# davidesantangelo/krep

Hardware: AMD Instinct MI355X
Metric: GB/s scanned (literal scan, match offsets produced), haystack resident in HBM (higher is better)
Workload: dtype u8; 1 GPU; literal8: 8-byte case-sensitive literal 'Sherlock', ~1e-4 matches/byte, offsets tracked; 32 GiB per GPU (BASELINE.json configs[1]); pattern=Sherlock, bytes_per_gpu=34359738368, matches=3436005, parallelism=contiguous shards x1, start-offset ownership, 1 RCCL all-reduce of counts

## Files before the change

### krep_amd/csrc/kg_literal_dma.hip

```cpp
#include <hip/hip_runtime.h>
#include <algorithm>
#include <atomic>
#include <cstdlib>
#include "kg_common.h"
#include "kg_device.h"
#include "kg_internal.h"
#include "kg_tickets.h"

namespace kg {

namespace {

constexpr u32 kDmaPark = 80;
constexpr u32 kDmaRing = 2u * kSegBytes;
constexpr u32 kDmaTail = 256u;
constexpr u32 kDmaWaveLds = kDmaRing + kDmaTail;
constexpr u32 kOpHits = 768;
constexpr u32 kOpTk = 32;
static_assert(kOpHits * 4u + kOpTk * 12u <= kDmaPark * 44u, "the one-pass mode's static LDS stays within the staging mode's (two workgroups per CU)");
static_assert(kOpTk <= 64u, "one lane per parked ticket picks its prefix up");
}
uint32_t lit_dma_one_pass_list() { return kOpHits; }

template <int KIND, bool MASKED, bool CI, bool ONEP>
__global__ __launch_bounds__(kBlock, 2) void lit_scan_dma(const LitArgs a, u64 *__restrict__ agg, const u64 *__restrict__ pref, const u64 n_tickets)
{
    extern __shared__ __attribute__((aligned(16))) uint8_t d_smem[];
    __shared__ u64 s_info_all[kWavesPerBlk][ONEP ? 1u : kDmaPark];
    __shared__ __attribute__((aligned(16))) unsigned short s_slots_all[kWavesPerBlk][ONEP ? 8u : kDmaPark * 16u];
    __shared__ u32 s_unit_all[kWavesPerBlk][ONEP ? 1u : kDmaPark];
    __shared__ u32 s_hits_all[kWavesPerBlk][ONEP ? kOpHits : 1u];
    __shared__ u32 s_tk_all[kWavesPerBlk][ONEP ? 3u * kOpTk : 1u];
    const u32 lane = lane_id();
    const u32 wave = __builtin_amdgcn_readfirstlane(threadIdx.x >> 6);
    if (ONEP && wave == 0)
    {
        u64 r = 1;
        if (lane == 0)
            r = __hip_atomic_fetch_add(&a.ctr->pad[0], 1ull, __ATOMIC_RELAXED, __HIP_MEMORY_SCOPE_AGENT);
        if (rfl64(r) == 0ull)
        {
            tk_resolve(agg, const_cast<u64 *>(pref), n_tickets, a.ctr, lane);
            return;
        }
    }
    u32 *s_hits = s_hits_all[wave];
    u32 *s_tk = s_tk_all[wave];
    uint8_t *ring = d_smem + wave * kDmaWaveLds;
    uint8_t *tailb = ring + kDmaRing;
    u64 *s_info = s_info_all[wave];
    unsigned short *s_slots = s_slots_all[wave];
    u32 *s_unit = s_unit_all[wave];
    const u32 ring_lds = (u32)(size_t)(__attribute__((address_space(3))) uint8_t *)ring;

    const bool want_pos = (a.flags & F_POS) != 0;
    const bool ww = (a.flags & F_WW) != 0;
    const u64 hi_match = (a.own_hi < a.text_len - a.m + 1) ? a.own_hi : (a.text_len - a.m + 1);
    constexpr u64 kUnitBytes = (u64)kRoundsBig * kSegBytes;
    const u64 n_units = a.num_tiles * kWavesPerBlk;

    const bool park = want_pos && a.stage_cap >= 16u && a.stage_cap <= 128u && (a.stage_cap & 7u) == 0u && n_units < (1ull << 32);
    const u32 park_max = park ? kDmaPark * 16u / a.stage_cap : 0u;
    u32 n_park = 0;
    auto flush_parked = [&]() __attribute__((always_inline)) {
        for (u32 i = lane; i < n_park; i += 64u)
        {
            const u64 u = s_unit[i];
            a.unitinfo[u] = s_info[i];
            if (s_info[i] & kUiCountMask)
            {
                uint4 *dst = reinterpret_cast<uint4 *>(reinterpret_cast<unsigned short *>(a.stage) + u * (u64)a.stage_cap);
                const uint4 *src = reinterpret_cast<const uint4 *>(&s_slots[i * a.stage_cap]);
                const u32 c = (u32)(s_info[i] & kUiCountMask), nv = ((c < a.stage_cap ? c : a.stage_cap) + 7u) >> 3;
                for (u32 q = 0; q < nv; ++q)
                    dst[q] = src[q];
            }
        }
        n_park = 0;
    };

    const u32 tk_units = a.upt ? a.upt : 1u;
    u64 static_next = (u64)blockIdx.x * kWavesPerBlk + wave;
    auto next_ticket = [&]() -> u64 {
        if (a.upt)
        {
            return wave_fetch_add(&a.ctr->ticket, 1ull, lane) * (u64)a.upt;
        }
        const u64 u = static_next;
        static_next += (u64)gridDim.x * kWavesPerBlk;
        return u;
    };
    auto issue_round = [&](u64 seg, u32 buf) -> bool {
        if (seg + kSegBytes > a.text_len)
            return false;
        const uint8_t *src = a.text + seg + lane * 16u;
        uint8_t *dst = ring + buf * kSegBytes;
#pragma unroll
        for (int j = 0; j < kCells; ++j)
            __builtin_amdgcn_global_load_lds((const __attribute__((address_space(1))) void *)(src + j * kCellBytes),
                                             (__attribute__((address_space(3))) void *)(dst + j * kCellBytes), 16, 0, 2 );
        return true;
    };
    auto issue_tail = [&](u64 at) -> bool {
        if (at + kDmaTail > a.text_len)
            return false;
        __builtin_amdgcn_global_load_lds((const __attribute__((address_space(1))) void *)(a.text + at + lane * 4u),
                                         (__attribute__((address_space(3))) void *)tailb, 4, 0, 0);
        return true;
    };

    u32 hp = 0;
    u32 used = 0;
    u32 n_tkp = 0;
    bool overflowed = false;
    auto hwrap = [](const u32 x) -> u32 { return x >= kOpHits ? x - kOpHits : x; };
    auto flush_records = [&](const u32 n_out) __attribute__((always_inline)) {
        u64 pfx = 0;
        if (lane < n_out)
            pfx = tk_wait_prefix_lane(pref, (u64)s_tk[3u * lane], a.ctr);
        for (u32 i = 0; i < n_out; ++i)
        {
            const u32 t = __builtin_amdgcn_readfirstlane(s_tk[3u * i]), cnt = __builtin_amdgcn_readfirstlane(s_tk[3u * i + 1u]),
                      at = __builtin_amdgcn_readfirstlane(s_tk[3u * i + 2u]);
            const u64 first = ((u64)(u32)__builtin_amdgcn_readlane((u32)(pfx >> 32), i) << 32) | (u32)__builtin_amdgcn_readlane((u32)pfx, i);
            const u64 tbase = a.global_base + a.anchor + (u64)t * ((u64)tk_units * kUnitBytes);
            const u32 pad = (u32)(first & 7ull);
            for (u32 q = lane; q < cnt + pad; q += 64u)
            {
                if (q < pad)
                    continue;
                const u32 e = q - pad;
                const u64 idx = first + e;
                if (idx < a.pos_cap)
                {
                    const u64 st = tbase + s_hits[hwrap(at + e)], en = st + a.m;
                    typedef u32 u32x4 __attribute__((ext_vector_type(4)));
                    const u32x4 rec = {(u32)st, (u32)(st >> 32), (u32)en, (u32)(en >> 32)};
                    __builtin_nontemporal_store(rec, reinterpret_cast<u32x4 *>(a.positions + 2 * idx));
                }
            }
            used -= cnt;
        }
        if (n_out < n_tkp)
        {
            const u32 t = s_tk[3u * n_out], cnt = s_tk[3u * n_out + 1u], at = s_tk[3u * n_out + 2u];
            if (lane == 0)
            {
                s_tk[0] = t;
                s_tk[1] = cnt;
                s_tk[2] = at;
            }
        }
        n_tkp -= n_out;
    };

    u64 acc_total = 0;
    u32 pf_cells = 0;
    u32 wcnt = 0;
    auto stage_hit = [&](u64 unit, u32 idx, u32 rel) __attribute__((always_inline)) {
        if (ONEP)
        {
            if (idx < kOpHits - used)
                s_hits[hwrap(hp + idx)] = rel;
        }
        else if (idx < a.stage_cap)
        {
            unsigned short *slot = park ? &s_slots[n_park * a.stage_cap] : reinterpret_cast<unsigned short *>(a.stage) + unit * (u64)a.stage_cap;
            slot[idx] = (unsigned short)rel;
        }
    };
    auto publish = [&](u64 unit) __attribute__((always_inline)) {
        if (ONEP)
            return;
        acc_total += wcnt;
        if (want_pos)
        {
            if (lane == 0)
            {
                const u64 info = (u64)wcnt | (wcnt ? (kLnHead | kLnTail) : 0ull);
                if (park)
                {
                    s_info[n_park] = info;
                    s_unit[n_park] = (u32)unit;
                }
                else
                    a.unitinfo[unit] = info;
                if (wcnt > a.stage_cap)
                {
                    atomicAdd(&a.ctr->overflow_units, 1ull);
                    atomicMax(&a.ctr->max_unit_count, (u64)wcnt);
                }
            }
            if (park && ++n_park == park_max)
                flush_parked();
        }
        wcnt = 0;
    };
    auto end_ticket = [&](u32 t) __attribute__((always_inline)) {
        if (lane == 0)
            __hip_atomic_store(&agg[t], (u64)wcnt | kTkReady, __ATOMIC_RELAXED, __HIP_MEMORY_SCOPE_AGENT);
        u32 fresh = 0;
        if (wcnt > kOpHits - used)
            overflowed = true;
        else if (wcnt)
        {
            if (lane == 0)
            {
                s_tk[3u * n_tkp] = t;
                s_tk[3u * n_tkp + 1u] = wcnt;
                s_tk[3u * n_tkp + 2u] = hp;
            }
            ++n_tkp;
            hp = hwrap(hp + wcnt);
            used += wcnt;
            fresh = 1;
        }
        wcnt = 0;
        if ((n_tkp == kOpTk || used > kOpHits / 2u) && n_tkp > fresh)
            flush_records(n_tkp - fresh);
    };
    auto exact = [&](u32 A0, u32 A4) -> bool {
        const u32 e0 = CI ? (A0 | a.l0) : A0;
        bool h = (KIND == 4 && MASKED) ? (((e0 ^ a.p0) & a.k0) == 0u) : (e0 == a.p0);
        if (KIND >= 8)
        {
            const u32 e4 = CI ? (A4 | a.l1) : A4;
            h = h && ((KIND == 8 && MASKED) ? (((e4 ^ a.p1) & a.k1) == 0u) : (e4 == a.p1));
        }
        return h;
    };
    auto owned = [&](u64 p) -> bool { return p >= a.own_lo && p < hi_match && !(p >= a.excl_lo && p < a.excl_hi); };
    auto word_ok = [&](u64 p) -> bool {
        if (p > 0 && p != a.ww_exempt_left && is_wordc(a.text[p - 1]))
            return false;
        if (p + a.m < a.text_len && is_wordc(a.text[p + a.m]))
            return false;
        return true;
    };
    auto boundary = [&](u64 seg_prev, u64 unit, u32 r_prev, u32 c0, u32 c1, u32 n0, u32 n1) __attribute__((always_inline)) {
        {
            const u32 f = 0x01010101u * ((CI ? (a.p0 | 0x20u) : a.p0) & 0xffu);
            const u32 y0 = (CI ? (c0 | 0x20202020u) : c0) ^ f, y1 = (CI ? (c1 | 0x20202020u) : c1) ^ f;
            if (((((y0 - 0x01010101u) & ~y0) | ((y1 - 0x01010101u) & ~y1)) & 0x80808080u) == 0u)
                return;
        }
        const u32 q = lane & 7u, sh = q & 3u;
        const bool up = (q >> 2) != 0u;
        const u32 lo = up ? c1 : c0, mid = up ? n0 : c1, hi = up ? n1 : n0;
        const u32 A0 = __builtin_amdgcn_alignbyte(mid, lo, sh), A4 = __builtin_amdgcn_alignbyte(hi, mid, sh);
        const u64 p = seg_prev + (kSegBytes - 8u) + q;
        bool h = lane < 8u && q + a.m > 8u && exact(A0, A4) && owned(p);
        if (ww && __ballot(h))
            h = h && word_ok(p);
        const u64 bm = __ballot(h);
        if (bm)
        {
            if (h && want_pos)
                stage_hit(unit, wcnt + mbcnt64(bm), r_prev * kSegBytes + (kSegBytes - 8u) + q);
            wcnt += (u32)__popcll(bm);
        }
    };

    u64 u0 = next_ticket();
    bool dma_cur = u0 < n_units && issue_round(a.anchor + u0 * kUnitBytes, 0u);
    while (u0 < n_units)
    {
        const u32 nun = (u32)((n_units - u0 < (u64)tk_units) ? (n_units - u0) : (u64)tk_units), nr = nun * (u32)kRoundsBig;
        const u64 tbase = a.anchor + u0 * kUnitBytes;
        u64 u_next = ~0ull;
        bool tail_ok = false;
        u32 c0 = 0, c1 = 0;
        bool deferred = false;
#pragma unroll 1
        for (u32 g = 0; g < nr; ++g)
        {
            const u64 seg = tbase + (u64)g * kSegBytes, unit = u0 + (g >> 2);
            const u32 r = g & 3u;
            bool dma_nx = false, tail_now = false;
            asm volatile("s_waitcnt lgkmcnt(0)" ::: "memory");
            if (g + 1u < nr)
                dma_nx = issue_round(seg + kSegBytes, (g + 1u) & 1u);
            else
            {
                u_next = next_ticket();
                if (u_next < n_units)
                    dma_nx = issue_round(a.anchor + u_next * kUnitBytes, (g + 1u) & 1u);
            }
            if (g + 2u == nr)
                tail_ok = tail_now = issue_tail(tbase + (u64)nr * kSegBytes);
            if (dma_cur)
            {
                if (dma_nx && tail_now)
                    asm volatile("s_waitcnt vmcnt(9)" ::: "memory");
                else if (dma_nx)
                    asm volatile("s_waitcnt vmcnt(8)" ::: "memory");
                else if (tail_now)
                    asm volatile("s_waitcnt vmcnt(1)" ::: "memory");
                else
                    asm volatile("s_waitcnt vmcnt(0)" ::: "memory");
            }
            const bool interior = seg >= a.own_lo && seg + kSegBytes <= hi_match && (seg + kSegBytes <= a.excl_lo || seg >= a.excl_hi);
            uint4 vv[kCells];
            uint2 nn[kCells];
            if (dma_cur)
            {
                typedef u32 v4 __attribute__((ext_vector_type(4)));
                typedef u32 v2 __attribute__((ext_vector_type(2)));
                const u32 addr = ring_lds + (g & 1u) * kSegBytes + lane * 16u;
                v4 x[kCells];
                v2 y[kCells];
#pragma unroll
                for (int j = 0; j < kCells; ++j)
                {
                    asm volatile("ds_read_b128 %0, %1 offset:%2" : "=v"(x[j]) : "v"(addr), "n"(j * (int)kCellBytes));
                    asm volatile("ds_read_b64 %0, %1 offset:%2" : "=v"(y[j]) : "v"(addr), "n"(j * (int)kCellBytes + 16));
                }
                asm volatile("s_waitcnt lgkmcnt(0)"
                             : "+v"(x[0]), "+v"(x[1]), "+v"(x[2]), "+v"(x[3]), "+v"(x[4]), "+v"(x[5]), "+v"(x[6]), "+v"(x[7]), "+v"(y[0]), "+v"(y[1]),
                               "+v"(y[2]), "+v"(y[3]), "+v"(y[4]), "+v"(y[5]), "+v"(y[6]), "+v"(y[7])
                             :
                             : "memory");
#pragma unroll
                for (int j = 0; j < kCells; ++j)
                {
                    vv[j] = make_uint4(x[j].x, x[j].y, x[j].z, x[j].w);
                    nn[j] = make_uint2(y[j].x, y[j].y);
                }
            }
            else
            {
#pragma unroll
                for (int j = 0; j < kCells; ++j)
                {
                    const W6 w = load_window_guarded(a.text, a.text_len, seg + (u64)j * kCellBytes + (u64)lane * 16u);
                    vv[j] = make_uint4(w.v[0], w.v[1], w.v[2], w.v[3]);
                    nn[j] = make_uint2(w.v[4], w.v[5]);
                }
            }
            if (deferred)
            {
                boundary(seg - kSegBytes, u0 + ((g - 1u) >> 2), ONEP ? g - 1u : (g - 1u) & 3u, c0, c1, __builtin_amdgcn_readfirstlane(vv[0].x),
                         __builtin_amdgcn_readfirstlane(vv[0].y));
                deferred = false;
                if (r == 0u)
                    publish(unit - 1u);
            }
            __builtin_amdgcn_sched_barrier(0);
#pragma unroll
            for (int j = 0; j < kCells; ++j)
            {
                const u64 lbase = seg + (u64)j * kCellBytes + (u64)lane * 16u;
                const u32 D[6] = {vv[j].x, vv[j].y, vv[j].z, vv[j].w, nn[j].x, nn[j].y};
                auto A = [&](int k) -> u32 {
                    return ((k & 3) == 0) ? D[k >> 2] : __builtin_amdgcn_alignbyte(D[(k >> 2) + 1], D[k >> 2], (u32)(k & 3));
                };
                u32 Dq[6];
#pragma unroll
                for (int w = 0; w < 6; ++w)
                    Dq[w] = CI ? (D[w] | 0x20202020u) : D[w];
                auto Aq = [&](int k) -> u32 {
                    return ((k & 3) == 0) ? Dq[k >> 2] : __builtin_amdgcn_alignbyte(Dq[(k >> 2) + 1], Dq[k >> 2], (u32)(k & 3));
                };
                const u32 p0q = CI ? (a.p0 | 0x20202020u) : a.p0;
                if (a.prefilter)
                {
                    u32 z = 0;
#pragma unroll
                    for (int w = 0; w < 4; ++w)
                    {
                        const u32 y = Dq[w] ^ a.prefilter;
                        z |= (y - 0x01010101u) & ~y;
                    }
                    if (!__ballot((z & 0x80808080u) != 0u))
                        continue;
                    ++pf_cells;
                }
                bool c[16];
                u64 any = 0;
#pragma unroll
                for (int k = 0; k < 16; ++k)
                {
                    const u32 x = Aq(k);
                    c[k] = (KIND == 4 && MASKED) ? (((x ^ p0q) & a.k0) == 0u) : (x == p0q);
                    any |= __ballot(c[k]);
                }
                if (!any)
                    continue;
                u32 m16 = 0;
#pragma unroll
                for (int k = 0; k < 16; ++k)
                    if (__ballot(c[k]))
                        m16 |= (c[k] && exact(A(k), A(k + 4))) ? (1u << k) : 0u;
                if (dma_cur && j == kCells - 1 && lane == 63u)
                    m16 &= (1u << (17u - a.m)) - 1u;
                if (!interior)
                {
                    auto clip = [&](u64 lo, u64 hi) -> u32 {
                        const u32 klo = lo > lbase ? (u32)((lo - lbase) < 16 ? (lo - lbase) : 16) : 0u;
                        const u32 khi = hi > lbase ? (u32)((hi - lbase) < 16 ? (hi - lbase) : 16) : 0u;
                        return khi > klo ? (((1u << khi) - 1u) & ~((1u << klo) - 1u)) : 0u;
                    };
                    m16 &= clip(a.own_lo, hi_match) & ~clip(a.excl_lo, a.excl_hi);
                }
                if (ww && __ballot(m16 != 0u))
                {
                    const u32 below = __shfl_up(D[3], 1);
                    auto pick = [&](u32 i) -> u32 {
                        const u32 q = i >> 2;
                        const u32 w = q == 0u ? below : q == 1u ? D[0] : q == 2u ? D[1] : q == 3u ? D[2] : q == 4u ? D[3] : q == 5u ? D[4] : D[5];
                        return (w >> (8u * (i & 3u))) & 0xffu;
                    };
                    const bool edge = dma_cur && j == kCells - 1 && lane == 63u;
                    u32 rest = m16;
                    while (rest)
                    {
                        const u32 k = __builtin_ctz(rest);
                        rest &= rest - 1u;
                        const u64 p = lbase + k;
                        bool bad;
                        if (edge || (lane == 0u && k == 0u))
                            bad = !word_ok(p);
                        else
                            bad = (p != a.ww_exempt_left && is_wordc(pick(k + 3u))) || is_wordc(pick(k + a.m + 4u));
                        if (bad)
                            m16 &= ~(1u << k);
                    }
                }
                if (!__ballot(m16 != 0u))
                    continue;
                const u32 cnt = __popc(m16);
                u32 idx = wcnt, tot = 0;
                auto plane = [&](int b) {
                    const u64 bm = __ballot((cnt >> b) & 1u);
                    idx += mbcnt64(bm) << b;
                    tot += (u32)__popcll(bm) << b;
                };
                plane(0);
                plane(1);
                if (__ballot(cnt > 3u))
                {
                    plane(2);
                    plane(3);
                    plane(4);
                }
                wcnt += tot;
                if (want_pos)
                {
                    const u32 rel0 = ((ONEP ? g : r) * (u32)kCells + (u32)j) * kCellBytes + lane * 16u;
                    u32 rest = m16;
                    while (rest)
                    {
                        const u32 k = __builtin_ctz(rest);
                        rest &= rest - 1u;
                        stage_hit(unit, idx++, rel0 + k);
                    }
                }
            }
            if (dma_cur)
            {
                c0 = __builtin_amdgcn_readlane(vv[kCells - 1].z, 63);
                c1 = __builtin_amdgcn_readlane(vv[kCells - 1].w, 63);
                deferred = true;
            }
            if (g + 1u == nr)
            {
                if (deferred)
                {
                    u32 n0 = 0, n1 = 0;
                    if (tail_ok)
                    {
                        typedef u32 v2 __attribute__((ext_vector_type(2)));
                        v2 t;
                        const u32 taddr = ring_lds + kDmaRing;
                        asm volatile("ds_read_b64 %0, %1\n\ts_waitcnt lgkmcnt(0)" : "=v"(t) : "v"(taddr) : "memory");
                        n0 = __builtin_amdgcn_readfirstlane(t.x);
                        n1 = __builtin_amdgcn_readfirstlane(t.y);
                    }
                    else
                    {
                        const W6 w = load_window_guarded(a.text, a.text_len, seg + kSegBytes);
                        n0 = __builtin_amdgcn_readfirstlane(w.v[0]);
                        n1 = __builtin_amdgcn_readfirstlane(w.v[1]);
                    }
                    boundary(seg, unit, ONEP ? g : r, c0, c1, n0, n1);
                    deferred = false;
                }
                if (ONEP)
                    end_ticket((u32)u0 / tk_units);
                else
                    publish(unit);
            }
            else if (!deferred && r == 3u)
                publish(unit);
            dma_cur = dma_nx;
        }
        u0 = u_next;
    }
    if (!ONEP && park && n_park)
        flush_parked();
    if (ONEP && n_tkp)
        flush_records(n_tkp);
    if (ONEP && overflowed && lane == 0)
        atomicAdd(&a.ctr->overflow_units, 1ull);
    if (lane == 0 && acc_total)
        atomicAdd(&a.ctr->total, acc_total);
    if (lane == 0 && pf_cells)
        atomicAdd(&a.ctr->candidates, (u64)pf_cells);
}

__global__ __launch_bounds__(256) void dma_byte_look(const uint8_t *text, u64 lo, u32 n_cells, u32 b4, u32 fold, unsigned long long *out)
{
    const u32 lane = lane_id();
    const u32 wave = blockIdx.x * 4u + (threadIdx.x >> 6), n_waves = gridDim.x * 4u;
    u32 cnt = 0;
    for (u32 c = wave; c < n_cells; c += n_waves)
    {
        const uint4 v = *reinterpret_cast<const uint4 *>(text + lo + (u64)c * kCellBytes + lane * 16u);
        const u32 d[4] = {v.x, v.y, v.z, v.w};
        u32 z = 0;
#pragma unroll
        for (int w = 0; w < 4; ++w)
        {
            const u32 y = (d[w] | fold) ^ b4;
            z |= (y - 0x01010101u) & ~y;
        }
        if (__ballot((z & 0x80808080u) != 0u))
            ++cnt;
    }
    if (lane == 0 && cnt)
        atomicAdd(out, (u64)cnt);
}
hipError_t launch_dma_byte_look(const uint8_t *text, uint64_t lo, uint32_t n_cells, uint32_t prefilter, bool ci, unsigned long long *out, hipStream_t st)
{
    hipLaunchKernelGGL(dma_byte_look, dim3(256), dim3(256), 0, st, text, (u64)lo, n_cells, prefilter, ci ? 0x20202020u : 0u, out);
    return hipGetLastError();
}

std::atomic<uint64_t> g_lit_dma_launches{0};
std::atomic<uint64_t> g_lit_dma1p_launches{0};
std::atomic<uint64_t> g_lit_dma1p_failovers{0};
int g_lit_dma1p_force_grid = 0;

template <int KIND, bool MASKED, bool CI, bool ONEP>
static hipError_t dma_launch4(const LitArgs &a, u64 *agg, const u64 *pref, u64 n_tickets, u32 num_cu, hipStream_t st)
{
    constexpr u32 lds = kWavesPerBlk * kDmaWaveLds;
    if (const hipError_t e = grant_dynamic_lds<&lit_scan_dma<KIND, MASKED, CI, ONEP>>((int)lds); e != hipSuccess)
        return e;
    static const u32 bpc = [] { const char *e = getenv("KREP_GPU_LIT_DMA_BLOCKS_PER_CU"); return e && atoi(e) > 0 ? (u32)atoi(e) : 2u; }();
    u32 grid = (u32)std::min<u64>(a.num_tiles, (u64)num_cu * bpc);
    if (ONEP && g_lit_dma1p_force_grid > 0)
        grid = std::min<u32>(grid, (u32)g_lit_dma1p_force_grid);
    hipLaunchKernelGGL((lit_scan_dma<KIND, MASKED, CI, ONEP>), dim3(grid ? grid : 1), dim3(kBlock), lds, st, a, agg, pref, n_tickets);
    g_lit_dma_launches.fetch_add(1, std::memory_order_relaxed);
    if (ONEP)
        g_lit_dma1p_launches.fetch_add(1, std::memory_order_relaxed);
    return hipGetLastError();
}
template <int KIND, bool MASKED, bool ONEP>
static hipError_t dma_launch2(const LitArgs &a, u64 *agg, const u64 *pref, u64 n_tickets, u32 num_cu, hipStream_t st)
{
    return (a.flags & F_CI) ? dma_launch4<KIND, MASKED, true, ONEP>(a, agg, pref, n_tickets, num_cu, st)
                            : dma_launch4<KIND, MASKED, false, ONEP>(a, agg, pref, n_tickets, num_cu, st);
}
template <bool ONEP>
static hipError_t dma_launch1(const LitArgs &a, u64 *agg, const u64 *pref, u64 n_tickets, u32 num_cu, hipStream_t st)
{
    if (a.m < 4)
        return dma_launch2<4, true, ONEP>(a, agg, pref, n_tickets, num_cu, st);
    if (a.m == 4)
        return dma_launch2<4, false, ONEP>(a, agg, pref, n_tickets, num_cu, st);
    if (a.m < 8)
        return dma_launch2<8, true, ONEP>(a, agg, pref, n_tickets, num_cu, st);
    return dma_launch2<8, false, ONEP>(a, agg, pref, n_tickets, num_cu, st);
}

bool literal_dma_eligible(const LitArgs &a)
{
    return !getenv("KREP_GPU_LIT_NO_DMA") && a.prefilter != 0u && a.m >= 2 && a.m <= 8 && a.rounds == (u32)kRoundsBig && !(a.flags & F_LINES) && !a.emit_mode &&
           (a.upt >= 4 || getenv("KREP_GPU_LIT_DMA_ALL")) && a.text_len >= 4u * kSegBytes;
}
hipError_t launch_literal_dma(const LitArgs &a, u32 num_cu, hipStream_t st)
{
    return dma_launch1<false>(a, nullptr, nullptr, 0, num_cu, st);
}
hipError_t launch_literal_dma_one_pass(const LitArgs &a, unsigned long long *d_agg, unsigned long long *d_pref, uint64_t n_tickets, u32 num_cu,
                                       hipStream_t st)
{
    const u64 n_units = a.num_tiles * kWavesPerBlk;
    if (!(a.flags & F_POS) || !a.upt || n_units >= (1ull << 32) || n_tickets != (n_units + a.upt - 1) / a.upt || (u64)a.upt * kRoundsBig * kSegBytes > (1ull << 31))
        return hipErrorInvalidValue;
    return dma_launch1<true>(a, d_agg, d_pref, n_tickets, num_cu, st);
}

}
```

Measured before the change: 6780 GB/s.

## Generalize the DMA LDS ring to NBUF buffers with templated occupancy shapes

Turns the hard-wired double-buffered LDS ring of the DMA literal scan into an NBUF-deep ring. It issues NBUF-1 rounds ahead and uses counted vmcnt waits derived from the number of outstanding rounds. Ring depth and workgroups per CU become template parameters chosen at launch through environment variables, and a static check keeps each shape within the CU's LDS. The default (2 buffers, 2 WGs per CU) matches the old behaviour, so the change mainly enables deeper prefetch at lower occupancy when selected. The env var parsing now rejects unsupported blocks-per-CU values that the old code accepted, and the forced-grid override now applies outside one-pass mode too.

```diff
diff --git a/krep_amd/csrc/kg_literal_dma.hip b/krep_amd/csrc/kg_literal_dma.hip
--- a/krep_amd/csrc/kg_literal_dma.hip
+++ b/krep_amd/csrc/kg_literal_dma.hip
@@ -12,9 +12,32 @@
 namespace {
 
 constexpr u32 kDmaPark = 80;
-constexpr u32 kDmaRing = 2u * kSegBytes;
 constexpr u32 kDmaTail = 256u;
-constexpr u32 kDmaWaveLds = kDmaRing + kDmaTail;
+constexpr u32 dma_ring_bytes(int nbuf) { return (u32)nbuf * kSegBytes; }
+constexpr u32 dma_wave_lds(int nbuf) { return dma_ring_bytes(nbuf) + kDmaTail; }
+constexpr u32 kDmaStaticLds = (u32)kWavesPerBlk * kDmaPark * 44u;
+constexpr u32 kLdsPerCu = 160u << 10;
+constexpr bool dma_shape_fits(int nbuf, int wgs) { return (u32)wgs * ((u32)kWavesPerBlk * dma_wave_lds(nbuf) + kDmaStaticLds) <= kLdsPerCu; }
+constexpr u32 dma_wait_count(u32 rounds_behind, bool tail_behind) { return rounds_behind * (u32)kCells + (tail_behind ? 1u : 0u); }
+constexpr u32 kVmcntMax = 63u;
+template <u32 N> __device__ __forceinline__ void wait_vm()
+{
+    static_assert(N <= kVmcntMax, "s_waitcnt vmcnt holds 6 bits");
+    asm volatile("s_waitcnt vmcnt(%0)" ::"n"(N) : "memory");
+}
+template <int R> __device__ __forceinline__ void dma_wait(u32 rounds_behind, bool tail_behind)
+{
+    if (rounds_behind == (u32)R)
+    {
+        if (tail_behind)
+            wait_vm<dma_wait_count(R, true)>();
+        else
+            wait_vm<dma_wait_count(R, false)>();
+        return;
+    }
+    if constexpr (R > 0)
+        dma_wait<R - 1>(rounds_behind, tail_behind);
+}
 constexpr u32 kOpHits = 768;
 constexpr u32 kOpTk = 32;
 static_assert(kOpHits * 4u + kOpTk * 12u <= kDmaPark * 44u, "the one-pass mode's static LDS stays within the staging mode's (two workgroups per CU)");
@@ -22,9 +45,13 @@
 }
 uint32_t lit_dma_one_pass_list() { return kOpHits; }
 
-template <int KIND, bool MASKED, bool CI, bool ONEP>
-__global__ __launch_bounds__(kBlock, 2) void lit_scan_dma(const LitArgs a, u64 *__restrict__ agg, const u64 *__restrict__ pref, const u64 n_tickets)
-{
+template <int KIND, bool MASKED, bool CI, bool ONEP, int NBUF, int WGS>
+__global__ __launch_bounds__(kBlock, WGS) void lit_scan_dma(const LitArgs a, u64 *__restrict__ agg, const u64 *__restrict__ pref, const u64 n_tickets)
+{
+    static_assert(NBUF >= 2 && NBUF - 1 <= kRoundsBig, "a ticket's first NBUF - 1 rounds are issued ahead of it: it has at least a unit's");
+    static_assert(dma_wait_count(NBUF - 1, true) <= kVmcntMax, "the deepest counted wait fits the 6-bit counter");
+    static_assert(dma_shape_fits(NBUF, WGS), "resident workgroups x (rings + tail pieces + parked stores) fit the CU's 160 KiB of LDS");
+    constexpr u32 kDmaRing = dma_ring_bytes(NBUF), kDmaWaveLds = dma_wave_lds(NBUF);
     extern __shared__ __attribute__((aligned(16))) uint8_t d_smem[];
     __shared__ u64 s_info_all[kWavesPerBlk][ONEP ? 1u : kDmaPark];
     __shared__ __attribute__((aligned(16))) unsigned short s_slots_all[kWavesPerBlk][ONEP ? 8u : kDmaPark * 16u];
@@ -262,7 +289,13 @@
     };
 
     u64 u0 = next_ticket();
-    bool dma_cur = u0 < n_units && issue_round(a.anchor + u0 * kUnitBytes, 0u);
+    u32 cb = 0, fl = 0;
+    if (u0 < n_units)
+    {
+#pragma unroll
+        for (int k = 0; k < NBUF - 1; ++k)
+            fl |= issue_round(a.anchor + u0 * kUnitBytes + (u64)k * kSegBytes, (u32)k) ? (1u << k) : 0u;
+    }
     while (u0 < n_units)
     {
         const u32 nun = (u32)((n_units - u0 < (u64)tk_units) ? (n_units - u0) : (u64)tk_units), nr = nun * (u32)kRoundsBig;
@@ -276,29 +309,26 @@
         {
             const u64 seg = tbase + (u64)g * kSegBytes, unit = u0 + (g >> 2);
             const u32 r = g & 3u;
-            bool dma_nx = false, tail_now = false;
+            const bool dma_cur = (fl & 1u) != 0u;
             asm volatile("s_waitcnt lgkmcnt(0)" ::: "memory");
-            if (g + 1u < nr)
-                dma_nx = issue_round(seg + kSegBytes, (g + 1u) & 1u);
-            else
-            {
-                u_next = next_ticket();
-                if (u_next < n_units)
-                    dma_nx = issue_round(a.anchor + u_next * kUnitBytes, (g + 1u) & 1u);
-            }
-            if (g + 2u == nr)
-                tail_ok = tail_now = issue_tail(tbase + (u64)nr * kSegBytes);
+            {
+                const u32 h = g + (u32)(NBUF - 1), hb = cb ? cb - 1u : (u32)(NBUF - 1);
+                bool ok = false;
+                if (h < nr)
+                    ok = issue_round(tbase + (u64)h * kSegBytes, hb);
+                else
+                {
+                    if (h == nr)
+                        u_next = next_ticket();
+                    if (u_next < n_units)
+                        ok = issue_round(a.anchor + u_next * kUnitBytes + (u64)(h - nr) * kSegBytes, hb);
+                }
+                fl |= ok ? (1u << (NBUF - 1)) : 0u;
+            }
+            if (g + (u32)NBUF == nr)
+                tail_ok = issue_tail(tbase + (u64)nr * kSegBytes);
             if (dma_cur)
-            {
-                if (dma_nx && tail_now)
-                    asm volatile("s_waitcnt vmcnt(9)" ::: "memory");
-                else if (dma_nx)
-                    asm volatile("s_waitcnt vmcnt(8)" ::: "memory");
-                else if (tail_now)
-                    asm volatile("s_waitcnt vmcnt(1)" ::: "memory");
-                else
-                    asm volatile("s_waitcnt vmcnt(0)" ::: "memory");
-            }
+                dma_wait<NBUF - 1>((u32)__popc(fl >> 1), tail_ok && g + 1u != nr);
             const bool interior = seg >= a.own_lo && seg + kSegBytes <= hi_match && (seg + kSegBytes <= a.excl_lo || seg >= a.excl_hi);
             uint4 vv[kCells];
             uint2 nn[kCells];
@@ -306,7 +336,7 @@
             {
                 typedef u32 v4 __attribute__((ext_vector_type(4)));
                 typedef u32 v2 __attribute__((ext_vector_type(2)));
-                const u32 addr = ring_lds + (g & 1u) * kSegBytes + lane * 16u;
+                const u32 addr = ring_lds + cb * kSegBytes + lane * 16u;
                 v4 x[kCells];
                 v2 y[kCells];
 #pragma unroll
@@ -492,7 +522,8 @@
             }
             else if (!deferred && r == 3u)
                 publish(unit);
-            dma_cur = dma_nx;
+            fl >>= 1;
+            cb = cb + 1u == (u32)NBUF ? 0u : cb + 1u;
         }
         u0 = u_next;
     }
@@ -541,21 +572,38 @@
 std::atomic<uint64_t> g_lit_dma1p_failovers{0};
 int g_lit_dma1p_force_grid = 0;
 
-template <int KIND, bool MASKED, bool CI, bool ONEP>
-static hipError_t dma_launch4(const LitArgs &a, u64 *agg, const u64 *pref, u64 n_tickets, u32 num_cu, hipStream_t st)
-{
-    constexpr u32 lds = kWavesPerBlk * kDmaWaveLds;
-    if (const hipError_t e = grant_dynamic_lds<&lit_scan_dma<KIND, MASKED, CI, ONEP>>((int)lds); e != hipSuccess)
+#define KG_DMA_SHAPES(X) X(2, 2) X(2, 1) X(3, 1) X(4, 1)
+constexpr int kDmaDefaultRing = 2, kDmaDefaultWgs = 2;
+
+template <int KIND, bool MASKED, bool CI, bool ONEP, int NBUF, int WGS>
+static hipError_t dma_launch5(const LitArgs &a, u64 *agg, const u64 *pref, u64 n_tickets, u32 num_cu, hipStream_t st)
+{
+    constexpr u32 lds = kWavesPerBlk * dma_wave_lds(NBUF);
+    if (const hipError_t e = grant_dynamic_lds<&lit_scan_dma<KIND, MASKED, CI, ONEP, NBUF, WGS>>((int)lds); e != hipSuccess)
         return e;
-    static const u32 bpc = [] { const char *e = getenv("KREP_GPU_LIT_DMA_BLOCKS_PER_CU"); return e && atoi(e) > 0 ? (u32)atoi(e) : 2u; }();
-    u32 grid = (u32)std::min<u64>(a.num_tiles, (u64)num_cu * bpc);
-    if (ONEP && g_lit_dma1p_force_grid > 0)
+    u32 grid = (u32)std::min<u64>(a.num_tiles, (u64)num_cu * (u32)WGS);
+    if (g_lit_dma1p_force_grid > 0)
         grid = std::min<u32>(grid, (u32)g_lit_dma1p_force_grid);
-    hipLaunchKernelGGL((lit_scan_dma<KIND, MASKED, CI, ONEP>), dim3(grid ? grid : 1), dim3(kBlock), lds, st, a, agg, pref, n_tickets);
+    hipLaunchKernelGGL((lit_scan_dma<KIND, MASKED, CI, ONEP, NBUF, WGS>), dim3(grid ? grid : 1), dim3(kBlock), lds, st, a, agg, pref, n_tickets);
     g_lit_dma_launches.fetch_add(1, std::memory_order_relaxed);
     if (ONEP)
         g_lit_dma1p_launches.fetch_add(1, std::memory_order_relaxed);
     return hipGetLastError();
+}
+template <int KIND, bool MASKED, bool CI, bool ONEP>
+static hipError_t dma_launch4(const LitArgs &a, u64 *agg, const u64 *pref, u64 n_tickets, u32 num_cu, hipStream_t st)
+{
+    int ring = kDmaDefaultRing, wgs = kDmaDefaultWgs;
+    if (const char *e = getenv("KREP_GPU_LIT_DMA_RING"))
+        ring = atoi(e);
+    if (const char *e = getenv("KREP_GPU_LIT_DMA_BLOCKS_PER_CU"))
+        wgs = atoi(e);
+#define KG_DMA_CASE(R, W)      \
+    if (ring == R && wgs == W) \
+        return dma_launch5<KIND, MASKED, CI, ONEP, R, W>(a, agg, pref, n_tickets, num_cu, st);
+    KG_DMA_SHAPES(KG_DMA_CASE)
+#undef KG_DMA_CASE
+    return hipErrorInvalidValue;
 }
 template <int KIND, bool MASKED, bool ONEP>
 static hipError_t dma_launch2(const LitArgs &a, u64 *agg, const u64 *pref, u64 n_tickets, u32 num_cu, hipStream_t st)
```

Result: no change. 6747 GB/s (-0.5%).
